# colmap/glomap

Measured on NVIDIA H100. Metric: observations/sec per BA LM-iteration, higher is better.
Workload: dtype f64

## Files before the change

### glomap_b200/csrc/ba_kernels.cuh

```cuda
#pragma once
#include "common.cuh"
#include "pcg.cuh"

namespace b200 {

constexpr int kCamRec = 8;
constexpr int kIntrRec = 8;
constexpr double kZEps = 1e-12;
constexpr int kSeg = 256;
constexpr int kIntrSmem = 16;
constexpr int kJpDoubles = 6;
constexpr int kSensorRec = 16;

struct BAView {
  int C, P, K;
  long long N;
  int n_tiles;
  int n_segs;
  int min_views;
  const int* obs_cam;
  const int* obs_pt;
  const double2* obs_xy;
  const unsigned* pt_begin;
  const int* tile_pt_begin;
// ... 22 lines not shown
  double* Dc;
};

__device__ __forceinline__ void huber(double s, double a, double& rho0, double& rho1) {
  const double b = a * a;
  if (s > b) {
    const double r = sqrt(s);
    rho0 = 2.0 * a * r - b;
    rho1 = fmax(2.2250738585072014e-308, a / r);
  } else {
    rho0 = s;
    rho1 = 1.0;
  }
}

__device__ __forceinline__ void project_jac(const double* __restrict__ ir, double x, double y, double z, double& px,
                                            double& py, double J[6]) {
  const double iz = 1.0 / z;
  const double u = x * iz, v = y * iz;
  const double fx = ir[0], fy = ir[1], cx = ir[2], cy = ir[3], k1 = ir[4], k2 = ir[5];
  const double r2 = u * u + v * v;
  const double d = 1.0 + r2 * (k1 + k2 * r2);
  const double dd = k1 + 2.0 * k2 * r2;
  px = fx * u * d + cx;
  py = fy * v * d + cy;
  const double a00 = d + 2.0 * u * u * dd, a01 = 2.0 * u * v * dd, a11 = d + 2.0 * v * v * dd;
  J[0] = fx * a00 * iz;
  J[1] = fx * a01 * iz;
  J[2] = -fx * iz * (a00 * u + a01 * v);
  J[3] = fy * a01 * iz;
  J[4] = fy * a11 * iz;
  J[5] = -fy * iz * (a01 * u + a11 * v);
}
__device__ __forceinline__ void project_only(const double* __restrict__ ir, double x, double y, double z, double& px,
                                             double& py) {
  const double iz = 1.0 / z;
  const double u = x * iz, v = y * iz;
  const double r2 = u * u + v * v;
  const double d = 1.0 + r2 * (ir[4] + ir[5] * r2);
  px = ir[0] * u * d + ir[2];
  py = ir[1] * v * d + ir[3];
}

struct ObsLin {
  double Jr[6], Jt[6], Jp[6], r[2], rho0;
  double u, v, w;
  bool valid;
};

__device__ __forceinline__ int cam_rec_intr(const double4& t4) { return (int)(__double_as_longlong(t4.w) >> 8); }

__device__ __forceinline__ void sensor_apply(const double* __restrict__ sr, double& x, double& y, double& z) {
  const double a = sr[0] * x + sr[1] * y + sr[2] * z + sr[9];
  const double b = sr[3] * x + sr[4] * y + sr[5] * z + sr[10];
  const double c = sr[6] * x + sr[7] * y + sr[8] * z + sr[11];
  x = a; y = b; z = c;
// ... 59 lines not shown
  for (int a = 0; a < 2; ++a) {
    const double j0 = J[3 * a], j1 = J[3 * a + 1], j2 = J[3 * a + 2];
    o.Jr[3 * a + 0] = rvar ? -2.0 * (j1 * rz - j2 * ry) : 0.0;
    o.Jr[3 * a + 1] = rvar ? -2.0 * (j2 * rx - j0 * rz) : 0.0;
    o.Jr[3 * a + 2] = rvar ? -2.0 * (j0 * ry - j1 * rx) : 0.0;
  }
#pragma unroll
  for (int a = 0; a < 2; ++a)
#pragma unroll
    for (int b = 0; b < 3; ++b) o.Jp[3 * a + b] = J[3 * a] * R[b] + J[3 * a + 1] * R[3 + b] + J[3 * a + 2] * R[6 + b];
}

struct ObsCore {
  double J[6], e[2], rho0, rho1, RX[3], R[9];
  double uv[2];
  bool valid;
};
__device__ __forceinline__ void obs_core(const double4& q4, const double4& t4, const double* __restrict__ ir,
                                         const double* __restrict__ sr, double X0, double X1, double X2, double2 xy,
                                         double huber_a, ObsCore& o) {
  const double q[4] = {q4.x, q4.y, q4.z, q4.w};
  quat_to_R(q, o.R);
  o.RX[0] = o.R[0] * X0 + o.R[1] * X1 + o.R[2] * X2;
  o.RX[1] = o.R[3] * X0 + o.R[4] * X1 + o.R[5] * X2;
  o.RX[2] = o.R[6] * X0 + o.R[7] * X1 + o.R[8] * X2;
  double xc = o.RX[0] + t4.x, yc = o.RX[1] + t4.y, zc = o.RX[2] + t4.z;
  if (sr) sensor_apply(sr, xc, yc, zc);
  o.valid = zc > kZEps;
  if (!o.valid) {
#pragma unroll
    for (int k = 0; k < 6; ++k) o.J[k] = 0.0;
    o.e[0] = o.e[1] = 0.0;
    o.rho0 = 0.0;
    o.rho1 = 0.0;
    o.uv[0] = o.uv[1] = 0.0;
    return;
  }
  double px, py;
  project_jac(ir, xc, yc, zc, px, py, o.J);
  o.uv[0] = xc / zc;
  o.uv[1] = yc / zc;
  if (sr) {
#pragma unroll
    for (int a = 0; a < 2; ++a) {
      const double j0 = o.J[3 * a], j1 = o.J[3 * a + 1], j2 = o.J[3 * a + 2];
      o.J[3 * a] = j0 * sr[0] + j1 * sr[3] + j2 * sr[6];
      o.J[3 * a + 1] = j0 * sr[1] + j1 * sr[4] + j2 * sr[7];
      o.J[3 * a + 2] = j0 * sr[2] + j1 * sr[5] + j2 * sr[8];
    }
  }
  o.e[0] = px - xy.x;
  o.e[1] = py - xy.y;
  const double s = o.e[0] * o.e[0] + o.e[1] * o.e[1];
  const double b = huber_a * huber_a;
  if (s > b) {
    const double t = rsqrt(s);
    o.rho1 = fmax(2.2250738585072014e-308, huber_a * t);
    o.rho0 = 2.0 * huber_a * (s * t) - b;
  } else {
    o.rho0 = s;
    o.rho1 = 1.0;
  }
}
__device__ __forceinline__ void obs_point_blocks(const ObsCore& o, double Jp[6], double A[6], double b[3]) {
#pragma unroll
  for (int a = 0; a < 2; ++a)
#pragma unroll
    for (int c = 0; c < 3; ++c) Jp[3 * a + c] = o.J[3 * a] * o.R[c] + o.J[3 * a + 1] * o.R[3 + c] + o.J[3 * a + 2] * o.R[6 + c];
  const double s0 = o.rho1 * Jp[0], s1 = o.rho1 * Jp[1], s2 = o.rho1 * Jp[2];
  const double s3 = o.rho1 * Jp[3], s4 = o.rho1 * Jp[4], s5 = o.rho1 * Jp[5];
  A[0] = s0 * Jp[0] + s3 * Jp[3];
  A[1] = s0 * Jp[1] + s3 * Jp[4];
  A[2] = s0 * Jp[2] + s3 * Jp[5];
  A[3] = s1 * Jp[1] + s4 * Jp[4];
  A[4] = s1 * Jp[2] + s4 * Jp[5];
  A[5] = s2 * Jp[2] + s5 * Jp[5];
  b[0] = s0 * o.e[0] + s3 * o.e[1];
// ... 672 lines not shown
    atomicAdd(&cscal[3], a3);
    atomicAdd(&cscal[4], a4);
  }
}


constexpr int kMaxBlockDof = 5;

struct IntrVarRec {
  int col0;
  int mb;
  int pidx[kMaxBlockDof];
  int pad;
};

__device__ __forceinline__ void intr_param_jac(const double* __restrict__ ir, int pidx, double u, double v, double w,
                                               double& jx, double& jy) {
  const int model = (int)ir[6];
  const double r2 = u * u + v * v;
  const double d = 1.0 + r2 * (ir[4] + ir[5] * r2);
  jx = 0.0;
  jy = 0.0;
  if (model == 1) {
    if (pidx == 0) jx = u;
    else if (pidx == 1) jy = v;
    else if (pidx == 2) jx = 1.0;
    else jy = 1.0;
  } else {
    if (pidx == 0) { jx = u * d; jy = v * d; }
    else if (pidx == 1) jx = 1.0;
    else if (pidx == 2) jy = 1.0;
    else if (pidx == 3) { jx = ir[0] * u * r2; jy = ir[1] * v * r2; }
    else { jx = ir[0] * u * r2 * r2; jy = ir[1] * v * r2 * r2; }
  }
  jx *= w;
  jy *= w;
}

__global__ void __launch_bounds__(256) ba_colsum(int rows, int ncol, const double* __restrict__ part,
                                                 double* __restrict__ out) {
  __shared__ double scratch[32];
  const int c = blockIdx.x;
  double a = 0.0;
  for (int r = threadIdx.x; r < rows; r += blockDim.x) a += part[(size_t)r * ncol + c];
  a = block_sum(a, scratch);
  if (threadIdx.x == 0) out[c] = a;
}

// ... 2 lines not shown
```

### glomap_b200/csrc/ba_kernels_ext.cuh

```cuda
#pragma once
#include "ba_kernels_v3.cuh"

namespace b200 {

struct ExtView {
  int C, K, S;
  const IntrVarRec* ivar;
  const unsigned char* sensor_var;
};

template <bool WK, bool WS>
struct ObsFull {
  double Jr[6], Jt[6], Jp[6], r[2], rho0;
  double Jk[WK ? 2 : 1][kMaxBlockDof];
  double Jsr[WS ? 6 : 1], Jst[WS ? 6 : 1];
  bool valid;
};

template <bool WK, bool WS>
__device__ __forceinline__ void obs_full(const double4& q4, const double4& t4, const double* __restrict__ ir,
                                         const IntrVarRec& iv, const double* __restrict__ sr, bool svar, double X0,
                                         double X1, double X2, double2 xy, double huber_a, ObsFull<WK, WS>& o) {
  const int mask = (int)(__double_as_longlong(t4.w) & 0xff);
  const double q[4] = {q4.x, q4.y, q4.z, q4.w};
// ... 35 lines not shown
#pragma unroll
      for (int a = 0; a < 2; ++a) {
        const double j0 = J[3 * a], j1 = J[3 * a + 1], j2 = J[3 * a + 2];
        o.Jsr[WS ? 3 * a + 0 : 0] = -2.0 * (j1 * a2 - j2 * a1);
        o.Jsr[WS ? 3 * a + 1 : 0] = -2.0 * (j2 * a0 - j0 * a2);
        o.Jsr[WS ? 3 * a + 2 : 0] = -2.0 * (j0 * a1 - j1 * a0);
        o.Jst[WS ? 3 * a + 0 : 0] = j0;
        o.Jst[WS ? 3 * a + 1 : 0] = j1;
        o.Jst[WS ? 3 * a + 2 : 0] = j2;
      }
    }
  }
  if (WK) {
#pragma unroll
    for (int j = 0; j < kMaxBlockDof; ++j)
      if (j < iv.mb) intr_param_jac(ir, iv.pidx[j], u, v, w, o.Jk[0][j], o.Jk[WK ? 1 : 0][j]);
  }
  if (sr) {
#pragma unroll
    for (int a = 0; a < 2; ++a) {
      const double j0 = J[3 * a], j1 = J[3 * a + 1], j2 = J[3 * a + 2];
      J[3 * a] = j0 * sr[0] + j1 * sr[3] + j2 * sr[6];
      J[3 * a + 1] = j0 * sr[1] + j1 * sr[4] + j2 * sr[7];
      J[3 * a + 2] = j0 * sr[2] + j1 * sr[5] + j2 * sr[8];
    }
  }
  const bool tvar = !(mask & 2), rvar = !(mask & 1);
#pragma unroll
  for (int a = 0; a < 2; ++a) {
    const double j0 = J[3 * a], j1 = J[3 * a + 1], j2 = J[3 * a + 2];
    if (tvar) { o.Jt[3 * a] = j0; o.Jt[3 * a + 1] = j1; o.Jt[3 * a + 2] = j2; }
// ... 391 lines not shown
```

### glomap_b200/csrc/ba_kernels_v2.cuh

```cuda
#pragma once
#include "ba_kernels.cuh"
#include "pcg.cuh"

namespace b200 {

struct BAViewV2 {
  const double* Ap;
  double* z4;
  const double* pts4;
  double* Ufk = nullptr;
  const IntrVarRec* ivar = nullptr;
  int C = 0;
};

template <int NK>
__device__ __forceinline__ void obs_intr_rows(const ObsCore& o, const double* __restrict__ ir, const IntrVarRec& iv,
                                              const double Jp[6], double Jk[2][NK > 0 ? NK : 1],
                                              double B[NK > 0 ? 3 * NK : 1]) {
#pragma unroll
  for (int j = 0; j < NK; ++j) {
    double jx = 0.0, jy = 0.0;
    if (j < iv.mb) intr_param_jac(ir, iv.pidx[j], o.uv[0], o.uv[1], 1.0, jx, jy);
    if (!o.valid) jx = jy = 0.0;
    Jk[0][j] = jx;
    Jk[1][j] = jy;
#pragma unroll
    for (int c = 0; c < 3; ++c) B[3 * j + c] = o.rho1 * (Jp[c] * jx + Jp[3 + c] * jy);
  }
}

constexpr int kXqStride = 8;
__global__ void ba2_pack_x(int C, const double* __restrict__ x, const double* __restrict__ cam_rec,
                           double* __restrict__ xp) {
  const int c = blockIdx.x * blockDim.x + threadIdx.x;
  if (c >= C) return;
  const double* r = cam_rec + (size_t)c * kCamRec;
  const double q[4] = {r[0], r[1], r[2], r[3]};
  double R[9];
  quat_to_R(q, R);
  const double* xc = x + (size_t)c * 6;
  double* o = xp + (size_t)c * kXqStride;
#pragma unroll
  for (int k = 0; k < 3; ++k) {
// ... 40 lines not shown
__global__ void ba2_pad_points(int P, const double* __restrict__ points, double* __restrict__ pts4) {
  const int p = blockIdx.x * blockDim.x + threadIdx.x;
  if (p >= P) return;
  const double x = points[3 * (size_t)p], y = points[3 * (size_t)p + 1], z = points[3 * (size_t)p + 2];
  st_rec32(pts4 + 4 * (size_t)p, x, y, z, 0.0);
}

template <int NK>
__global__ void __launch_bounds__(128, NK > 0 ? 3 : B200_LC_MIN_CTAS) ba2_linearize_cams(BAView v, BAViewV2 v2, const double* __restrict__ cam_rec,
                                                         const double* __restrict__ intr_rec, double huber_a) {
  const int warp = (blockIdx.x * blockDim.x + threadIdx.x) >> 5;
  const int lane = threadIdx.x & 31;
  if (warp >= v.n_segs) return;
  const int cam = v.seg_cam[warp];
  const int b = v.seg_begin[warp], e = v.seg_end[warp];
  const double4 q4c = ld_rec32(cam_rec + (size_t)cam * kCamRec);
  const double4 t4c = ld_rec32(cam_rec + (size_t)cam * kCamRec + 4);
  const double* irc = intr_rec + (size_t)v.seg_intr[warp] * kIntrRec;
  const double* src = sensor_of_seg(v, warp);
  double U[21], g[6];
#pragma unroll
  for (int k = 0; k < 21; ++k) U[k] = 0.0;
#pragma unroll
  for (int k = 0; k < 6; ++k) g[k] = 0.0;
  const int cmask = (int)(__double_as_longlong(t4c.w) & 0xff);
  const bool tvar = !(cmask & 2), rvar = !(cmask & 1);
  constexpr int NKK = NK > 0 ? NK : 1;
  const int blk = v.seg_intr[warp];
  IntrVarRec iv{};
  if (NK > 0) iv = v2.ivar[blk];
  double Ukk[NKK * (NKK + 1) / 2], gk[NKK], Ufk[6][NKK];
#pragma unroll
  for (int k = 0; k < NKK * (NKK + 1) / 2; ++k) Ukk[k] = 0.0;
#pragma unroll
  for (int k = 0; k < NKK; ++k) {
    gk[k] = 0.0;
#pragma unroll
    for (int i2 = 0; i2 < 6; ++i2) Ufk[i2][k] = 0.0;
  }
  const double* __restrict__ pts4 = v2.pts4;
// ... 6 lines not shown
    if (i + 32 < e) pt_nxt = ld_stream(v.pt_c + i + 32);
    xy = ld_stream(v.xy_c + i);
    Xc = ld_rec32(pts4 + 4 * (size_t)pt0);
  }
  for (; i < e; i += 32) {
    double4 Xn = Xc;
    double2 xyn = xy;
    int pt_nn = 0;
    if (i + 32 < e) {
      Xn = ld_rec32(pts4 + 4 * (size_t)pt_nxt);
      xyn = ld_stream(v.xy_c + i + 32);
    }
    if (i + 64 < e) pt_nn = ld_stream(v.pt_c + i + 64);
    const double X0 = Xc.x, X1 = Xc.y, X2 = Xc.z;
    ObsCore o;
    obs_core(q4c, t4c, irc, src, X0, X1, X2, xy, huber_a, o);
    double Jp[6], A[6], bo[3];
    obs_point_blocks(o, Jp, A, bo);
    double Jc[2][6];
#pragma unroll
    for (int a = 0; a < 2; ++a) {
      const double j0 = o.J[3 * a], j1 = o.J[3 * a + 1], j2 = o.J[3 * a + 2];
      Jc[a][0] = rvar ? -2.0 * (j1 * o.RX[2] - j2 * o.RX[1]) : 0.0;
      Jc[a][1] = rvar ? -2.0 * (j2 * o.RX[0] - j0 * o.RX[2]) : 0.0;
      Jc[a][2] = rvar ? -2.0 * (j0 * o.RX[1] - j1 * o.RX[0]) : 0.0;
      Jc[a][3] = tvar ? j0 : 0.0;
      Jc[a][4] = tvar ? j1 : 0.0;
      Jc[a][5] = tvar ? j2 : 0.0;
    }
    const double e0 = o.rho1 * o.e[0], e1 = o.rho1 * o.e[1];
    int idx = 0;
#pragma unroll
    for (int i2 = 0; i2 < 6; ++i2) {
      const double s0 = o.rho1 * Jc[0][i2], s1 = o.rho1 * Jc[1][i2];
#pragma unroll
      for (int j = i2; j < 6; ++j) U[idx++] += s0 * Jc[0][j] + s1 * Jc[1][j];
      g[i2] += Jc[0][i2] * e0 + Jc[1][i2] * e1;
    }
    if (NK > 0) {
      double Jk[2][NKK], Bo[3 * NKK];
      obs_intr_rows<NK>(o, irc, iv, Jp, Jk, Bo);
      int ik = 0;
#pragma unroll
      for (int a = 0; a < NK; ++a) {
        const double s0 = o.rho1 * Jk[0][a], s1 = o.rho1 * Jk[1][a];
#pragma unroll
        for (int c = a; c < NK; ++c) Ukk[ik++] += s0 * Jk[0][c] + s1 * Jk[1][c];
        gk[a] += Jk[0][a] * e0 + Jk[1][a] * e1;
#pragma unroll
        for (int i2 = 0; i2 < 6; ++i2) Ufk[i2][a] += Jc[0][i2] * s0 + Jc[1][i2] * s1;
      }
    }
    Xc = Xn; xy = xyn; pt_nxt = pt_nn;
  }
  if (NK > 0) {
    const size_t kb = (size_t)(v2.C + blk);
// ... 14 lines not shown
      }
    }
  }
#pragma unroll
  for (int k = 0; k < 21; ++k) {
    const double s = warp_sum(U[k]);
    if (lane == k && s != 0.0) atomicAdd(&v.U[(size_t)cam * 21 + k], s);
  }
#pragma unroll
  for (int k = 0; k < 6; ++k) {
    const double s = warp_sum(g[k]);
    if (lane == 21 + k && s != 0.0) atomicAdd(&v.gc[(size_t)cam * 6 + k], s);
  }
}

__global__ void __launch_bounds__(128) ba2_schur_diag(BAView v, BAViewV2 v2, const double* __restrict__ cam_rec,
                                                      const double* __restrict__ intr_rec, double huber_a) {
  const int warp = (blockIdx.x * blockDim.x + threadIdx.x) >> 5;
  const int lane = threadIdx.x & 31;
  if (warp >= v.n_segs) return;
  const int cam = v.seg_cam[warp];
  const int b = v.seg_begin[warp], e = v.seg_end[warp];
  const double4 q4c = ld_rec32(cam_rec + (size_t)cam * kCamRec);
  const double4 t4c = ld_rec32(cam_rec + (size_t)cam * kCamRec + 4);
  const double* irc = intr_rec + (size_t)v.seg_intr[warp] * kIntrRec;
  const double* src = sensor_of_seg(v, warp);
  double RR[6] = {0, 0, 0, 0, 0, 0}, RT[9] = {0, 0, 0, 0, 0, 0, 0, 0, 0}, TT[6] = {0, 0, 0, 0, 0, 0};
  int i = b + lane;
  int pt_nxt = 0;
  double2 xy = make_double2(0, 0), va = xy, vb = xy, vc = xy;
  double4 Xc = make_double4(0, 0, 0, 0);
  if (i < e) {
    const int pt0 = ld_stream(v.pt_c + i);
    if (i + 32 < e) pt_nxt = ld_stream(v.pt_c + i + 32);
    xy = ld_stream(v.xy_c + i);
    Xc = ld_rec32(v2.pts4 + 4 * (size_t)pt0);
    const double2* vp = reinterpret_cast<const double2*>(v.Vinv + (size_t)pt0 * 6);
    va = vp[0]; vb = vp[1]; vc = vp[2];
  }
  for (; i < e; i += 32) {
    double4 Xn = Xc;
    double2 xyn = xy, van = va, vbn = vb, vcn = vc;
    int pt_nn = 0;
    if (i + 32 < e) {
      Xn = ld_rec32(v2.pts4 + 4 * (size_t)pt_nxt);
      xyn = ld_stream(v.xy_c + i + 32);
      const double2* vp = reinterpret_cast<const double2*>(v.Vinv + (size_t)pt_nxt * 6);
      van = vp[0]; vbn = vp[1]; vcn = vp[2];
    }
    if (i + 64 < e) pt_nn = ld_stream(v.pt_c + i + 64);
    const double X[3] = {Xc.x, Xc.y, Xc.z};
    ObsCore o;
    obs_core(q4c, t4c, irc, src, X[0], X[1], X[2], xy, huber_a, o);
    double Jp[6], A[6], bo[3];
    obs_point_blocks(o, Jp, A, bo);
    const double vi[6] = {va.x, va.y, vb.x, vb.y, vc.x, vc.y};
    const double Ac0[3] = {A[0], A[1], A[2]}, Ac1[3] = {A[1], A[3], A[4]}, Ac2[3] = {A[2], A[4], A[5]};
    double T0[3], T1[3], T2[3];
    sym3_mul(vi, Ac0, T0);
    sym3_mul(vi, Ac1, T1);
    sym3_mul(vi, Ac2, T2);
    double N[3][3];
    {
      double c0[3], c1[3], c2[3];
      sym3_mul(A, T0, c0);
      sym3_mul(A, T1, c1);
      sym3_mul(A, T2, c2);
#pragma unroll
      for (int r = 0; r < 3; ++r) { N[r][0] = c0[r]; N[r][1] = c1[r]; N[r][2] = c2[r]; }
    }
    double P[3][3];
#pragma unroll
    for (int c = 0; c < 3; ++c) {
      const double n0 = N[0][c], n1 = N[1][c], n2 = N[2][c];
      P[0][c] = 2.0 * (X[1] * n2 - X[2] * n1);
      P[1][c] = 2.0 * (X[2] * n0 - X[0] * n2);
      P[2][c] = 2.0 * (X[0] * n1 - X[1] * n0);
    }
    double PK[3][3];
#pragma unroll
    for (int r = 0; r < 3; ++r) {
      PK[r][0] = P[r][1] * X[2] - P[r][2] * X[1];
      PK[r][1] = -P[r][0] * X[2] + P[r][2] * X[0];
      PK[r][2] = P[r][0] * X[1] - P[r][1] * X[0];
    }
// ... 1 lines not shown
    RR[3] += -2.0 * PK[1][1]; RR[4] += -2.0 * PK[1][2]; RR[5] += -2.0 * PK[2][2];
#pragma unroll
    for (int r = 0; r < 3; ++r)
#pragma unroll
      for (int c = 0; c < 3; ++c) RT[3 * r + c] += P[r][c];
    TT[0] += N[0][0]; TT[1] += N[0][1]; TT[2] += N[0][2]; TT[3] += N[1][1]; TT[4] += N[1][2]; TT[5] += N[2][2];
    Xc = Xn; xy = xyn; va = van; vb = vbn; vc = vcn; pt_nxt = pt_nn;
  }
#pragma unroll
  for (int k = 0; k < 6; ++k) RR[k] = warp_sum(RR[k]);
#pragma unroll
  for (int k = 0; k < 9; ++k) RT[k] = warp_sum(RT[k]);
#pragma unroll
  for (int k = 0; k < 6; ++k) TT[k] = warp_sum(TT[k]);
  if (lane == 0) {
    const int mask = (int)(__double_as_longlong(t4c.w) & 0xff);
    const double q[4] = {q4c.x, q4c.y, q4c.z, q4c.w};
    double R[9];
    quat_to_R(q, R);
    double M[6][6];
    const double rr[3][3] = {{RR[0], RR[1], RR[2]}, {RR[1], RR[3], RR[4]}, {RR[2], RR[4], RR[5]}};
    const double tt[3][3] = {{TT[0], TT[1], TT[2]}, {TT[1], TT[3], TT[4]}, {TT[2], TT[4], TT[5]}};
    for (int r = 0; r < 3; ++r)
      for (int c = 0; c < 3; ++c) {
        M[r][c] = rr[r][c];
        M[3 + r][3 + c] = tt[r][c];
        M[r][3 + c] = RT[3 * r + c];
        M[3 + c][r] = RT[3 * r + c];
      }
    double T[6][6];
    for (int blk = 0; blk < 2; ++blk)
      for (int r = 0; r < 3; ++r)
        for (int c = 0; c < 6; ++c)
          T[3 * blk + r][c] = R[3 * r] * M[3 * blk][c] + R[3 * r + 1] * M[3 * blk + 1][c] + R[3 * r + 2] * M[3 * blk + 2][c];
// ... 194 lines not shown
  const bool pvalid = (int)(v.pt_begin[p + 1] - v.pt_begin[p]) >= v.min_views;
  *reinterpret_cast<double4*>(v2.z4 + 4 * (size_t)p) = pvalid ? make_double4(z[0], z[1], z[2], 0.0) : make_double4(0, 0, 0, 0);
}

template <int NK>
__global__ void __launch_bounds__(128, B200_PB_MIN_CTAS) ba2_pass_b(BAView v, BAViewV2 v2, const double* __restrict__ cam_rec,
                                                 const double* __restrict__ intr_rec, double huber_a,
                                                 double* __restrict__ y, const PcgCtl* __restrict__ ctl, int seg_lo,
                                                 int seg_hi) {
  if (ctl && ctl->done) return;
  const int warp = seg_lo + ((blockIdx.x * blockDim.x + threadIdx.x) >> 5);
  const int lane = threadIdx.x & 31;
  if (warp >= seg_hi) return;
  const int cam = v.seg_cam[warp];
  const int b = v.seg_begin[warp], e = v.seg_end[warp];
  const double4 q4c = ld_rec32(cam_rec + (size_t)cam * kCamRec);
  const double4 t4c = ld_rec32(cam_rec + (size_t)cam * kCamRec + 4);
  const int blk = v.seg_intr[warp];
  const double* irc = intr_rec + (size_t)blk * kIntrRec;
  const double* src = sensor_of_seg(v, warp);
  constexpr int NKK = NK > 0 ? NK : 1;
  IntrVarRec iv{};
  if (NK > 0) iv = v2.ivar[blk];
  double acc[6] = {0, 0, 0, 0, 0, 0};
  double accK[NKK];
#pragma unroll
  for (int k = 0; k < NKK; ++k) accK[k] = 0.0;
  const uint64_t keep = l2_policy_evict_last();
  int i = b + lane;
  int pt_nxt = 0;
  double4 X = make_double4(0, 0, 0, 0), z = X;
  double2 xy = make_double2(0, 0);
  if (i < e) {
    const int pt0 = ld_stream(v.pt_c + i);
    if (i + 32 < e) pt_nxt = ld_stream(v.pt_c + i + 32);
    X = ld_rec32(v2.pts4 + 4 * (size_t)pt0);
    z = ld_keep4(v2.z4 + 4 * (size_t)pt0, keep);
    xy = ld_stream(v.xy_c + i);
  }
  for (; i < e; i += 32) {
    double4 Xn = X, zn = z;
    double2 xyn = xy;
    int pt_nn = 0;
    if (i + 32 < e) {
      Xn = ld_rec32(v2.pts4 + 4 * (size_t)pt_nxt);
      zn = ld_keep4(v2.z4 + 4 * (size_t)pt_nxt, keep);
      xyn = ld_stream(v.xy_c + i + 32);
    }
    if (i + 64 < e) pt_nn = ld_stream(v.pt_c + i + 64);
    ObsCore o;
    obs_core(q4c, t4c, irc, src, X.x, X.y, X.z, xy, huber_a, o);
    double Jp[6], a[6], bo[3];
    obs_point_blocks(o, Jp, a, bo);
    const double w0 = a[0] * z.x + a[1] * z.y + a[2] * z.z;
    const double w1 = a[1] * z.x + a[3] * z.y + a[4] * z.z;
    const double w2 = a[2] * z.x + a[4] * z.y + a[5] * z.z;
    acc[0] += 2.0 * (X.y * w2 - X.z * w1);
    acc[1] += 2.0 * (X.z * w0 - X.x * w2);
    acc[2] += 2.0 * (X.x * w1 - X.y * w0);
    acc[3] += w0;
    acc[4] += w1;
    acc[5] += w2;
    if (NK > 0) {
      double Jk[2][NKK], Bo[3 * NKK];
      obs_intr_rows<NK>(o, irc, iv, Jp, Jk, Bo);
#pragma unroll
      for (int k = 0; k < NK; ++k) accK[k] += Bo[3 * k] * z.x + Bo[3 * k + 1] * z.y + Bo[3 * k + 2] * z.z;
    }
    X = Xn; z = zn; xy = xyn; pt_nxt = pt_nn;
  }
#pragma unroll
  for (int k = 0; k < 6; ++k) acc[k] = warp_sum(acc[k]);
  if (lane < 6) {
    const int mask = (int)(__double_as_longlong(t4c.w) & 0xff);
    const double q[4] = {q4c.x, q4c.y, q4c.z, q4c.w};
    double R[9];
    quat_to_R(q, R);
    const int bl = lane / 3, r = lane % 3;
    const bool fixed = bl == 0 ? (mask & 1) : (mask & 2);
    const double s = R[3 * r] * acc[3 * bl] + R[3 * r + 1] * acc[3 * bl + 1] + R[3 * r + 2] * acc[3 * bl + 2];
    if (!fixed && s != 0.0) atomicAdd(&y[(size_t)cam * 6 + lane], -s);
  }
  if (NK > 0) {
    const size_t kb = (size_t)(v2.C + blk);
#pragma unroll
    for (int k = 0; k < NK; ++k) {
      const double sk = warp_sum(accK[k]);
      if (lane == 0 && sk != 0.0) atomicAdd(&y[kb * 6 + k], -sk);
    }
  }
}

__global__ void ba2k_pack_xk(int C, const double* __restrict__ cam_rec, const double* __restrict__ x, double* __restrict__ xp,
                             const PcgCtl* __restrict__ ctl) {
  if (ctl && ctl->done) return;
  const int c = blockIdx.x * blockDim.x + threadIdx.x;
// ... 57 lines not shown
```

### glomap_b200/csrc/ba_kernels_v3.cuh

```cuda
#pragma once
#include "ba_kernels_v2.cuh"

namespace b200 {

constexpr int kEllWindow = 1024;
constexpr int kEllThreads = 128;

struct EllView {
  int n_groups;
  const int* row0;
  const int* pt;
  const int* len;
  const int* cam;
  const double2* xy;
  const unsigned short* sensor;
  double* A;
  double* B = nullptr;
};

template <class Sort>
__global__ void __launch_bounds__(kEllWindow) ell_sort_window(int P, int min_views, const unsigned* __restrict__ pt_begin,
                                                              int* __restrict__ ell_pt, int* __restrict__ ell_len,
                                                              int* __restrict__ ell_slot, int* __restrict__ group_rows) {
  __shared__ typename Sort::TempStorage tmp;
// ... 115 lines not shown
      obs_core(qA, tA, ir, sr, X0, X1, X2, xyA, huber_a, o);
      cost += 0.5 * o.rho0;
      if (points_var) {
        double Jp[6], A[6], b[3];
        obs_point_blocks(o, Jp, A, b);
        double* row = ell.A + ((size_t)r0 + j) * (6 * 32) + lane;
#pragma unroll
        for (int k = 0; k < 6; ++k) {
          st_stream(row + 32 * k, A[k]);
          V[k] += A[k];
        }
        gp[0] += b[0]; gp[1] += b[1]; gp[2] += b[2];
        if (NK > 0) {
          constexpr int NKK = NK > 0 ? NK : 1;
          double Jk[2][NKK], Bo[3 * NKK];
          obs_intr_rows<NK>(o, ir, ivar[blk], Jp, Jk, Bo);
          double* rowB = ell.B + ((size_t)r0 + j) * (3 * NK * 32) + lane;
#pragma unroll
          for (int k = 0; k < 3 * NK; ++k) st_stream(rowB + 32 * k, Bo[k]);
        }
      }
#if B200_E1_PIPE >= 2
      qA = qB; tA = tB; qB2 = qC; tB2 = tC; xyA = xyB; xyB = xyC; camC2 = camD;
#else
      qA = qB; tA = tB; xyA = xyB; xyB = xyC; camB = camC;
#endif
    }
#else
#pragma unroll 2
    for (int j = 0; j < nrow; ++j) {
      if (j >= mylen) continue;
// ... 9 lines not shown
      obs_core(q4, t4, ir, sr, X0, X1, X2, xy, huber_a, o);
      cost += 0.5 * o.rho0;
      if (points_var) {
        double Jp[6], A[6], b[3];
        obs_point_blocks(o, Jp, A, b);
        double* row = ell.A + ((size_t)r0 + j) * (6 * 32) + lane;
#pragma unroll
        for (int k = 0; k < 6; ++k) {
          st_stream(row + 32 * k, A[k]);
          V[k] += A[k];
        }
        gp[0] += b[0]; gp[1] += b[1]; gp[2] += b[2];
        if (NK > 0) {
          constexpr int NKK = NK > 0 ? NK : 1;
          double Jk[2][NKK], Bo[3 * NKK];
          obs_intr_rows<NK>(o, ir, ivar[blk], Jp, Jk, Bo);
          double* rowB = ell.B + ((size_t)r0 + j) * (3 * NK * 32) + lane;
#pragma unroll
          for (int k = 0; k < 3 * NK; ++k) st_stream(rowB + 32 * k, Bo[k]);
        }
      }
    }
#endif
    if (points_var && pt >= 0) {
#pragma unroll
      for (int k = 0; k < 6; ++k) v.V[6 * (size_t)pt + k] = V[k];
#pragma unroll
      for (int k = 0; k < 3; ++k) {
        v.gp[3 * (size_t)pt + k] = gp[k];
        gmax = fmax(gmax, fabs(gp[k]));
      }
// ... 180 lines not shown
```

### glomap_b200/csrc/common.cuh

```cuda
#pragma once
#include <cuda_runtime.h>
#include <stdint.h>
#include <stdio.h>

#include <string>

namespace b200 {

#ifndef B200_TILE
#define B200_TILE 128
#endif
#ifndef B200_K1_MIN_CTAS
#define B200_K1_MIN_CTAS 5
#endif
#ifndef B200_K3_MIN_CTAS
#define B200_K3_MIN_CTAS 8
#endif
#ifndef B200_PA_MIN_CTAS
#define B200_PA_MIN_CTAS 12
#endif
#ifndef B200_LC_MIN_CTAS
#define B200_LC_MIN_CTAS 3
#endif
#ifndef B200_PB_MIN_CTAS
#define B200_PB_MIN_CTAS 4
#endif
#ifndef B200_E1_MIN_CTAS
#define B200_E1_MIN_CTAS 4
#endif
#ifndef B200_E1_PIPE
#define B200_E1_PIPE 1
#endif
#ifndef B200_EA_MIN_CTAS
#define B200_EA_MIN_CTAS 8
#endif
#ifndef B200_EA2_MIN_CTAS
#define B200_EA2_MIN_CTAS 6
#endif
#ifndef B200_STREAM_HINTS
#define B200_STREAM_HINTS 1
// ... 283 lines not shown
```

### profiles/sass_excerpt.py

```python
#!/usr/bin/env python
import collections
import os
import re
import subprocess

ROOT = os.path.dirname(os.path.dirname(os.path.abspath(__file__)))
KERNELS = ["ba3_linearize_points", "ba2_linearize_cams", "ba3_pass_a", "ba2_pass_b", "ba2_schur_diag", "ba3_cost",
           "ba2_pcg_direction_pack", "pcg_update", "pcg_apply_diag", "bax_pass_b", "ba2k_cross", "gp_schur_pass", "ra_laplacian_csr",
           "ra2_laplacian_dot", "ra2_coarse", "p2p_allreduce_sum", "proc_undistort", "trk_hook"]
KEEP = re.compile(r"^(LDG|STG|LDS|STS|RED|ATOM|BAR|SHFL|DFMA|DMUL|DADD|MUFU|CCTL|UBLKCP|SYNCS|MEMBAR|ERRBAR|LDGSTS)")


def main():
    lib = os.path.join(ROOT, "glomap_b200", "libb200sfm.so")
    txt = subprocess.run(["cuobjdump", "-sass", lib], capture_output=True, text=True).stdout
    names = subprocess.run(["cu++filt"], input="\n".join(re.findall(r"Function : (\S+)", txt)), capture_output=True, text=True).stdout.split("\n")
    mangled = re.findall(r"Function : (\S+)", txt)
    demangle = dict(zip(mangled, names))
    cur, counts, totals = None, collections.defaultdict(collections.Counter), collections.Counter()
    for line in txt.splitlines():
        m = re.search(r"Function : (\S+)", line)
        if m:
            cur = demangle.get(m.group(1), m.group(1))
            continue
        m = re.search(r"/\*[0-9a-f]{4}\*/\s+(?:@!?U?P\d+\s+)?([A-Z0-9_.]+)", line)
        if m and cur:
            totals[cur] += 1
            op = m.group(1)
            if KEEP.match(op):
                counts[cur][op] += 1
    print("# SASS mnemonics of the hot kernels (cuobjdump -sass glomap_b200/libb200sfm.so, sm_90a)")
    print("# per kernel: total instructions, then the memory / synchronisation / FP64 mnemonics with their static counts")
    print("# (profiles/sass_excerpt.py regenerates this file; no tensor-core or TMA mnemonics are expected: FP64 streaming kernels)\n")
    for k in sorted(counts):
        if not any(re.search(r"\b" + re.escape(n) + r"\b", k) for n in KERNELS):
            continue
        ops = ", ".join(f"{o} x{c}" for o, c in counts[k].most_common(14))
        print(k[:200])
        print(f"    total {totals[k]} instructions: {ops}")


if __name__ == "__main__":
    main()
```

Baseline: 1.405 billion.

## Hoist per-segment rotation and factor projection Jacobian to cut FP64 work in BA kernels

```diff
diff --git a/glomap_b200/csrc/ba_kernels.cuh b/glomap_b200/csrc/ba_kernels.cuh
--- a/glomap_b200/csrc/ba_kernels.cuh
+++ b/glomap_b200/csrc/ba_kernels.cuh
@@ -60,32 +60,69 @@
   }
 }
 
+struct Intr {
+  double fx, fy, cx, cy, k1, k2;
+  int model;
+};
+__device__ __forceinline__ Intr ld_intr(const double* __restrict__ ir) {
+  return Intr{ir[0], ir[1], ir[2], ir[3], ir[4], ir[5], (int)ir[6]};
+}
+
+struct ProjJac {
+  double iz, u, v, m00, m01, m10, m11;
+};
+
+__device__ __forceinline__ void project_jac(const Intr& in, double x, double y, double z, double& px, double& py,
+                                            ProjJac& pj) {
+  const double iz = 1.0 / z;
+  const double u = x * iz, v = y * iz;
+  pj.iz = iz;
+  pj.u = u;
+  pj.v = v;
+  if (in.k1 == 0.0 && in.k2 == 0.0) {
+    px = in.fx * u + in.cx;
+    py = in.fy * v + in.cy;
+    pj.m00 = in.fx; pj.m01 = 0.0; pj.m10 = 0.0; pj.m11 = in.fy;
+  } else {
+    const double r2 = u * u + v * v;
+    const double d = 1.0 + r2 * (in.k1 + in.k2 * r2);
+    const double dd = in.k1 + 2.0 * in.k2 * r2;
+    px = in.fx * u * d + in.cx;
+    py = in.fy * v * d + in.cy;
+    const double a00 = d + 2.0 * u * u * dd, a01 = 2.0 * u * v * dd, a11 = d + 2.0 * v * v * dd;
+    pj.m00 = in.fx * a00; pj.m01 = in.fx * a01; pj.m10 = in.fy * a01; pj.m11 = in.fy * a11;
+  }
+}
+__device__ __forceinline__ void project_only(const Intr& in, double x, double y, double z, double& px, double& py) {
+  const double iz = 1.0 / z;
+  const double u = x * iz, v = y * iz;
+  if (in.k1 == 0.0 && in.k2 == 0.0) {
+    px = in.fx * u + in.cx;
+    py = in.fy * v + in.cy;
+  } else {
+    const double r2 = u * u + v * v;
+    const double d = 1.0 + r2 * (in.k1 + in.k2 * r2);
+    px = in.fx * u * d + in.cx;
+    py = in.fy * v * d + in.cy;
+  }
+}
+__device__ __forceinline__ void proj_jac_rows(const ProjJac& pj, double J[6]) {
+  J[0] = pj.m00 * pj.iz;
+  J[1] = pj.m01 * pj.iz;
+  J[2] = -(J[0] * pj.u + J[1] * pj.v);
+  J[3] = pj.m10 * pj.iz;
+  J[4] = pj.m11 * pj.iz;
+  J[5] = -(J[3] * pj.u + J[4] * pj.v);
+}
 __device__ __forceinline__ void project_jac(const double* __restrict__ ir, double x, double y, double z, double& px,
                                             double& py, double J[6]) {
-  const double iz = 1.0 / z;
-  const double u = x * iz, v = y * iz;
-  const double fx = ir[0], fy = ir[1], cx = ir[2], cy = ir[3], k1 = ir[4], k2 = ir[5];
-  const double r2 = u * u + v * v;
-  const double d = 1.0 + r2 * (k1 + k2 * r2);
-  const double dd = k1 + 2.0 * k2 * r2;
-  px = fx * u * d + cx;
-  py = fy * v * d + cy;
-  const double a00 = d + 2.0 * u * u * dd, a01 = 2.0 * u * v * dd, a11 = d + 2.0 * v * v * dd;
-  J[0] = fx * a00 * iz;
-  J[1] = fx * a01 * iz;
-  J[2] = -fx * iz * (a00 * u + a01 * v);
-  J[3] = fy * a01 * iz;
-  J[4] = fy * a11 * iz;
-  J[5] = -fy * iz * (a01 * u + a11 * v);
+  ProjJac pj;
+  project_jac(ld_intr(ir), x, y, z, px, py, pj);
+  proj_jac_rows(pj, J);
 }
 __device__ __forceinline__ void project_only(const double* __restrict__ ir, double x, double y, double z, double& px,
                                              double& py) {
-  const double iz = 1.0 / z;
-  const double u = x * iz, v = y * iz;
-  const double r2 = u * u + v * v;
-  const double d = 1.0 + r2 * (ir[4] + ir[5] * r2);
-  px = ir[0] * u * d + ir[2];
-  py = ir[1] * v * d + ir[3];
+  project_only(ld_intr(ir), x, y, z, px, py);
 }
 
 struct ObsLin {
@@ -175,13 +212,14 @@
 struct ObsCore {
   double J[6], e[2], rho0, rho1, RX[3], R[9];
   double uv[2];
+  ProjJac pj;
   bool valid;
 };
-__device__ __forceinline__ void obs_core(const double4& q4, const double4& t4, const double* __restrict__ ir,
-                                         const double* __restrict__ sr, double X0, double X1, double X2, double2 xy,
-                                         double huber_a, ObsCore& o) {
-  const double q[4] = {q4.x, q4.y, q4.z, q4.w};
-  quat_to_R(q, o.R);
+__device__ __forceinline__ void obs_core_R(const double R[9], const double4& t4, const Intr& in,
+                                           const double* __restrict__ sr, double X0, double X1, double X2, double2 xy,
+                                           double huber_a, ObsCore& o) {
+#pragma unroll
+  for (int k = 0; k < 9; ++k) o.R[k] = R[k];
   o.RX[0] = o.R[0] * X0 + o.R[1] * X1 + o.R[2] * X2;
   o.RX[1] = o.R[3] * X0 + o.R[4] * X1 + o.R[5] * X2;
   o.RX[2] = o.R[6] * X0 + o.R[7] * X1 + o.R[8] * X2;
@@ -195,10 +233,12 @@
     o.rho0 = 0.0;
     o.rho1 = 0.0;
     o.uv[0] = o.uv[1] = 0.0;
+    o.pj = ProjJac{0.0, 0.0, 0.0, 0.0, 0.0, 0.0, 0.0};
     return;
   }
   double px, py;
-  project_jac(ir, xc, yc, zc, px, py, o.J);
+  project_jac(in, xc, yc, zc, px, py, o.pj);
+  proj_jac_rows(o.pj, o.J);
   o.uv[0] = xc / zc;
   o.uv[1] = yc / zc;
   if (sr) {
@@ -222,6 +262,14 @@
     o.rho0 = s;
     o.rho1 = 1.0;
   }
+}
+__device__ __forceinline__ void obs_core(const double4& q4, const double4& t4, const double* __restrict__ ir,
+                                         const double* __restrict__ sr, double X0, double X1, double X2, double2 xy,
+                                         double huber_a, ObsCore& o) {
+  const double q[4] = {q4.x, q4.y, q4.z, q4.w};
+  double R[9];
+  quat_to_R(q, R);
+  obs_core_R(R, t4, ld_intr(ir), sr, X0, X1, X2, xy, huber_a, o);
 }
 __device__ __forceinline__ void obs_point_blocks(const ObsCore& o, double Jp[6], double A[6], double b[3]) {
 #pragma unroll
@@ -924,14 +972,13 @@
   int pad;
 };
 
-__device__ __forceinline__ void intr_param_jac(const double* __restrict__ ir, int pidx, double u, double v, double w,
+__device__ __forceinline__ void intr_param_jac(const Intr& in, int pidx, double u, double v, double w,
                                                double& jx, double& jy) {
-  const int model = (int)ir[6];
   const double r2 = u * u + v * v;
-  const double d = 1.0 + r2 * (ir[4] + ir[5] * r2);
+  const double d = 1.0 + r2 * (in.k1 + in.k2 * r2);
   jx = 0.0;
   jy = 0.0;
-  if (model == 1) {
+  if (in.model == 1) {
     if (pidx == 0) jx = u;
     else if (pidx == 1) jy = v;
     else if (pidx == 2) jx = 1.0;
@@ -940,8 +987,8 @@
     if (pidx == 0) { jx = u * d; jy = v * d; }
     else if (pidx == 1) jx = 1.0;
     else if (pidx == 2) jy = 1.0;
-    else if (pidx == 3) { jx = ir[0] * u * r2; jy = ir[1] * v * r2; }
-    else { jx = ir[0] * u * r2 * r2; jy = ir[1] * v * r2 * r2; }
+    else if (pidx == 3) { jx = in.fx * u * r2; jy = in.fy * v * r2; }
+    else { jx = in.fx * u * r2 * r2; jy = in.fy * v * r2 * r2; }
   }
   jx *= w;
   jy *= w;
diff --git a/glomap_b200/csrc/ba_kernels_ext.cuh b/glomap_b200/csrc/ba_kernels_ext.cuh
--- a/glomap_b200/csrc/ba_kernels_ext.cuh
+++ b/glomap_b200/csrc/ba_kernels_ext.cuh
@@ -73,7 +73,7 @@
   if (WK) {
 #pragma unroll
     for (int j = 0; j < kMaxBlockDof; ++j)
-      if (j < iv.mb) intr_param_jac(ir, iv.pidx[j], u, v, w, o.Jk[0][j], o.Jk[WK ? 1 : 0][j]);
+      if (j < iv.mb) intr_param_jac(ld_intr(ir), iv.pidx[j], u, v, w, o.Jk[0][j], o.Jk[WK ? 1 : 0][j]);
   }
   if (sr) {
 #pragma unroll
diff --git a/glomap_b200/csrc/ba_kernels_v2.cuh b/glomap_b200/csrc/ba_kernels_v2.cuh
--- a/glomap_b200/csrc/ba_kernels_v2.cuh
+++ b/glomap_b200/csrc/ba_kernels_v2.cuh
@@ -14,19 +14,64 @@
 };
 
 template <int NK>
-__device__ __forceinline__ void obs_intr_rows(const ObsCore& o, const double* __restrict__ ir, const IntrVarRec& iv,
-                                              const double Jp[6], double Jk[2][NK > 0 ? NK : 1],
-                                              double B[NK > 0 ? 3 * NK : 1]) {
+__device__ __forceinline__ void obs_intr_jac(const ObsCore& o, const Intr& in, const IntrVarRec& iv,
+                                             double Jk[2][NK > 0 ? NK : 1]) {
 #pragma unroll
   for (int j = 0; j < NK; ++j) {
     double jx = 0.0, jy = 0.0;
-    if (j < iv.mb) intr_param_jac(ir, iv.pidx[j], o.uv[0], o.uv[1], 1.0, jx, jy);
+    if (j < iv.mb) intr_param_jac(in, iv.pidx[j], o.uv[0], o.uv[1], 1.0, jx, jy);
     if (!o.valid) jx = jy = 0.0;
     Jk[0][j] = jx;
     Jk[1][j] = jy;
-#pragma unroll
-    for (int c = 0; c < 3; ++c) B[3 * j + c] = o.rho1 * (Jp[c] * jx + Jp[3 + c] * jy);
-  }
+  }
+}
+template <int NK>
+__device__ __forceinline__ void obs_intr_rows(const ObsCore& o, const Intr& in, const IntrVarRec& iv,
+                                              const double Jp[6], double Jk[2][NK > 0 ? NK : 1],
+                                              double B[NK > 0 ? 3 * NK : 1]) {
+  obs_intr_jac<NK>(o, in, iv, Jk);
+#pragma unroll
+  for (int j = 0; j < NK; ++j)
+#pragma unroll
+    for (int c = 0; c < 3; ++c) B[3 * j + c] = o.rho1 * (Jp[c] * Jk[0][j] + Jp[3 + c] * Jk[1][j]);
+}
+
+struct SegRec {
+  double R[9];
+  double4 t4;
+  Intr in;
+  const double* sr;
+};
+__device__ __forceinline__ void seg_records(const BAView& v, int seg, int cam, const double* __restrict__ cam_rec,
+                                            const double* __restrict__ intr_rec, SegRec& s) {
+  const double4 q4 = ld_rec32(cam_rec + (size_t)cam * kCamRec);
+  s.t4 = ld_rec32(cam_rec + (size_t)cam * kCamRec + 4);
+  s.in = ld_intr(intr_rec + (size_t)v.seg_intr[seg] * kIntrRec);
+  s.sr = sensor_of_seg(v, seg);
+  const double q[4] = {q4.x, q4.y, q4.z, q4.w};
+  quat_to_R(q, s.R);
+}
+__device__ __forceinline__ void to_sensor(const double* __restrict__ sr, double x[3]) {
+  if (!sr) return;
+  const double x0 = x[0], x1 = x[1], x2 = x[2];
+#pragma unroll
+  for (int k = 0; k < 3; ++k) x[k] = sr[3 * k] * x0 + sr[3 * k + 1] * x1 + sr[3 * k + 2] * x2;
+}
+__device__ __forceinline__ void cam_frame_jac(const ObsCore& o, const double r[3], double a[2], double w[3]) {
+  const ProjJac& p = o.pj;
+  const double t0 = r[0] - p.u * r[2], t1 = r[1] - p.v * r[2];
+  const double c = o.rho1 * p.iz;
+  a[0] = c * (p.m00 * t0 + p.m01 * t1);
+  a[1] = c * (p.m10 * t0 + p.m11 * t1);
+  const double s0 = p.iz * (p.m00 * a[0] + p.m10 * a[1]), s1 = p.iz * (p.m01 * a[0] + p.m11 * a[1]);
+  w[0] = s0;
+  w[1] = s1;
+  w[2] = -(p.u * s0 + p.v * s1);
+}
+__device__ __forceinline__ void rig_to_frame(const double* __restrict__ sr, double x[3]) {
+  const double x0 = x[0], x1 = x[1], x2 = x[2];
+#pragma unroll
+  for (int k = 0; k < 3; ++k) x[k] = sr[k] * x0 + sr[3 + k] * x1 + sr[6 + k] * x2;
 }
 
 constexpr int kXqStride = 8;
@@ -97,16 +142,14 @@
   if (warp >= v.n_segs) return;
   const int cam = v.seg_cam[warp];
   const int b = v.seg_begin[warp], e = v.seg_end[warp];
-  const double4 q4c = ld_rec32(cam_rec + (size_t)cam * kCamRec);
-  const double4 t4c = ld_rec32(cam_rec + (size_t)cam * kCamRec + 4);
-  const double* irc = intr_rec + (size_t)v.seg_intr[warp] * kIntrRec;
-  const double* src = sensor_of_seg(v, warp);
+  SegRec sg;
+  seg_records(v, warp, cam, cam_rec, intr_rec, sg);
   double U[21], g[6];
 #pragma unroll
   for (int k = 0; k < 21; ++k) U[k] = 0.0;
 #pragma unroll
   for (int k = 0; k < 6; ++k) g[k] = 0.0;
-  const int cmask = (int)(__double_as_longlong(t4c.w) & 0xff);
+  const int cmask = (int)(__double_as_longlong(sg.t4.w) & 0xff);
   const bool tvar = !(cmask & 2), rvar = !(cmask & 1);
   constexpr int NKK = NK > 0 ? NK : 1;
   const int blk = v.seg_intr[warp];
@@ -143,9 +186,7 @@
     if (i + 64 < e) pt_nn = ld_stream(v.pt_c + i + 64);
     const double X0 = Xc.x, X1 = Xc.y, X2 = Xc.z;
     ObsCore o;
-    obs_core(q4c, t4c, irc, src, X0, X1, X2, xy, huber_a, o);
-    double Jp[6], A[6], bo[3];
-    obs_point_blocks(o, Jp, A, bo);
+    obs_core_R(sg.R, sg.t4, sg.in, sg.sr, X0, X1, X2, xy, huber_a, o);
     double Jc[2][6];
 #pragma unroll
     for (int a = 0; a < 2; ++a) {
@@ -167,8 +208,8 @@
       g[i2] += Jc[0][i2] * e0 + Jc[1][i2] * e1;
     }
     if (NK > 0) {
-      double Jk[2][NKK], Bo[3 * NKK];
-      obs_intr_rows<NK>(o, irc, iv, Jp, Jk, Bo);
+      double Jk[2][NKK];
+      obs_intr_jac<NK>(o, sg.in, iv, Jk);
       int ik = 0;
 #pragma unroll
       for (int a = 0; a < NK; ++a) {
@@ -213,17 +254,15 @@
   }
 }
 
-__global__ void __launch_bounds__(128) ba2_schur_diag(BAView v, BAViewV2 v2, const double* __restrict__ cam_rec,
-                                                      const double* __restrict__ intr_rec, double huber_a) {
+__global__ void __launch_bounds__(128, B200_SD_MIN_CTAS) ba2_schur_diag(BAView v, BAViewV2 v2, const double* __restrict__ cam_rec,
+                                                                        const double* __restrict__ intr_rec, double huber_a) {
   const int warp = (blockIdx.x * blockDim.x + threadIdx.x) >> 5;
   const int lane = threadIdx.x & 31;
   if (warp >= v.n_segs) return;
   const int cam = v.seg_cam[warp];
   const int b = v.seg_begin[warp], e = v.seg_end[warp];
-  const double4 q4c = ld_rec32(cam_rec + (size_t)cam * kCamRec);
-  const double4 t4c = ld_rec32(cam_rec + (size_t)cam * kCamRec + 4);
-  const double* irc = intr_rec + (size_t)v.seg_intr[warp] * kIntrRec;
-  const double* src = sensor_of_seg(v, warp);
+  SegRec sg;
+  seg_records(v, warp, cam, cam_rec, intr_rec, sg);
   double RR[6] = {0, 0, 0, 0, 0, 0}, RT[9] = {0, 0, 0, 0, 0, 0, 0, 0, 0}, TT[6] = {0, 0, 0, 0, 0, 0};
   int i = b + lane;
   int pt_nxt = 0;
@@ -248,26 +287,42 @@
       van = vp[0]; vbn = vp[1]; vcn = vp[2];
     }
     if (i + 64 < e) pt_nn = ld_stream(v.pt_c + i + 64);
-    const double X[3] = {Xc.x, Xc.y, Xc.z};
     ObsCore o;
-    obs_core(q4c, t4c, irc, src, X[0], X[1], X[2], xy, huber_a, o);
-    double Jp[6], A[6], bo[3];
-    obs_point_blocks(o, Jp, A, bo);
+    obs_core_R(sg.R, sg.t4, sg.in, sg.sr, Xc.x, Xc.y, Xc.z, xy, huber_a, o);
+    double X[3] = {o.RX[0], o.RX[1], o.RX[2]};
+    to_sensor(sg.sr, X);
+    const ProjJac& pj = o.pj;
     const double vi[6] = {va.x, va.y, vb.x, vb.y, vc.x, vc.y};
-    const double Ac0[3] = {A[0], A[1], A[2]}, Ac1[3] = {A[1], A[3], A[4]}, Ac2[3] = {A[2], A[4], A[5]};
-    double T0[3], T1[3], T2[3];
-    sym3_mul(vi, Ac0, T0);
-    sym3_mul(vi, Ac1, T1);
-    sym3_mul(vi, Ac2, T2);
+    double e0[3] = {1.0, 0.0, -pj.u}, e1[3] = {0.0, 1.0, -pj.v};
+    if (sg.sr) {
+#pragma unroll
+      for (int c = 0; c < 3; ++c) {
+        e0[c] = sg.sr[c] - pj.u * sg.sr[6 + c];
+        e1[c] = sg.sr[3 + c] - pj.v * sg.sr[6 + c];
+      }
+    }
+    double l0[3], l1[3], t0[3], t1[3];
+#pragma unroll
+    for (int c = 0; c < 3; ++c) {
+      l0[c] = e0[0] * sg.R[c] + e0[1] * sg.R[3 + c] + e0[2] * sg.R[6 + c];
+      l1[c] = e1[0] * sg.R[c] + e1[1] * sg.R[3 + c] + e1[2] * sg.R[6 + c];
+    }
+    sym3_mul(vi, l0, t0);
+    sym3_mul(vi, l1, t1);
+    const double q00 = l0[0] * t0[0] + l0[1] * t0[1] + l0[2] * t0[2];
+    const double q01 = l0[0] * t1[0] + l0[1] * t1[1] + l0[2] * t1[2];
+    const double q11 = l1[0] * t1[0] + l1[1] * t1[1] + l1[2] * t1[2];
+    const double k00 = pj.m00 * pj.m00 + pj.m10 * pj.m10, k01 = pj.m00 * pj.m01 + pj.m10 * pj.m11,
+                 k11 = pj.m01 * pj.m01 + pj.m11 * pj.m11;
+    const double a00 = k00 * q00 + k01 * q01, a01 = k00 * q01 + k01 * q11;
+    const double a10 = k01 * q00 + k11 * q01, a11 = k01 * q01 + k11 * q11;
+    const double sc = o.rho1 * pj.iz * pj.iz, c2 = sc * sc;
+    const double h00 = c2 * (a00 * k00 + a01 * k01), h01 = c2 * (a00 * k01 + a01 * k11), h11 = c2 * (a10 * k01 + a11 * k11);
     double N[3][3];
-    {
-      double c0[3], c1[3], c2[3];
-      sym3_mul(A, T0, c0);
-      sym3_mul(A, T1, c1);
-      sym3_mul(A, T2, c2);
-#pragma unroll
-      for (int r = 0; r < 3; ++r) { N[r][0] = c0[r]; N[r][1] = c1[r]; N[r][2] = c2[r]; }
-    }
+    N[0][0] = h00; N[0][1] = N[1][0] = h01; N[1][1] = h11;
+    N[0][2] = N[2][0] = -(h00 * pj.u + h01 * pj.v);
+    N[1][2] = N[2][1] = -(h01 * pj.u + h11 * pj.v);
+    N[2][2] = -(N[0][2] * pj.u + N[1][2] * pj.v);
     double P[3][3];
 #pragma unroll
     for (int c = 0; c < 3; ++c) {
@@ -299,10 +354,12 @@
 #pragma unroll
   for (int k = 0; k < 6; ++k) TT[k] = warp_sum(TT[k]);
   if (lane == 0) {
-    const int mask = (int)(__double_as_longlong(t4c.w) & 0xff);
-    const double q[4] = {q4c.x, q4c.y, q4c.z, q4c.w};
-    double R[9];
-    quat_to_R(q, R);
+    const int mask = (int)(__double_as_longlong(sg.t4.w) & 0xff);
+    double R[9] = {1, 0, 0, 0, 1, 0, 0, 0, 1};
+    if (sg.sr) {
+      for (int r = 0; r < 3; ++r)
+        for (int c = 0; c < 3; ++c) R[3 * r + c] = sg.sr[3 * c + r];
+    }
     double M[6][6];
     const double rr[3][3] = {{RR[0], RR[1], RR[2]}, {RR[1], RR[3], RR[4]}, {RR[2], RR[4], RR[5]}};
     const double tt[3][3] = {{TT[0], TT[1], TT[2]}, {TT[1], TT[3], TT[4]}, {TT[2], TT[4], TT[5]}};
@@ -527,11 +584,9 @@
   if (warp >= seg_hi) return;
   const int cam = v.seg_cam[warp];
   const int b = v.seg_begin[warp], e = v.seg_end[warp];
-  const double4 q4c = ld_rec32(cam_rec + (size_t)cam * kCamRec);
-  const double4 t4c = ld_rec32(cam_rec + (size_t)cam * kCamRec + 4);
   const int blk = v.seg_intr[warp];
-  const double* irc = intr_rec + (size_t)blk * kIntrRec;
-  const double* src = sensor_of_seg(v, warp);
+  SegRec sg;
+  seg_records(v, warp, cam, cam_rec, intr_rec, sg);
   constexpr int NKK = NK > 0 ? NK : 1;
   IntrVarRec iv{};
   if (NK > 0) iv = v2.ivar[blk];
@@ -562,37 +617,41 @@
     }
     if (i + 64 < e) pt_nn = ld_stream(v.pt_c + i + 64);
     ObsCore o;
-    obs_core(q4c, t4c, irc, src, X.x, X.y, X.z, xy, huber_a, o);
-    double Jp[6], a[6], bo[3];
-    obs_point_blocks(o, Jp, a, bo);
-    const double w0 = a[0] * z.x + a[1] * z.y + a[2] * z.z;
-    const double w1 = a[1] * z.x + a[3] * z.y + a[4] * z.z;
-    const double w2 = a[2] * z.x + a[4] * z.y + a[5] * z.z;
-    acc[0] += 2.0 * (X.y * w2 - X.z * w1);
-    acc[1] += 2.0 * (X.z * w0 - X.x * w2);
-    acc[2] += 2.0 * (X.x * w1 - X.y * w0);
-    acc[3] += w0;
-    acc[4] += w1;
-    acc[5] += w2;
+    obs_core_R(sg.R, sg.t4, sg.in, sg.sr, X.x, X.y, X.z, xy, huber_a, o);
+    double P[3] = {o.RX[0], o.RX[1], o.RX[2]};
+    to_sensor(sg.sr, P);
+    double r[3] = {sg.R[0] * z.x + sg.R[1] * z.y + sg.R[2] * z.z,
+                   sg.R[3] * z.x + sg.R[4] * z.y + sg.R[5] * z.z,
+                   sg.R[6] * z.x + sg.R[7] * z.y + sg.R[8] * z.z};
+    to_sensor(sg.sr, r);
+    double a[2], w[3];
+    cam_frame_jac(o, r, a, w);
+    acc[0] += P[1] * w[2] - P[2] * w[1];
+    acc[1] += P[2] * w[0] - P[0] * w[2];
+    acc[2] += P[0] * w[1] - P[1] * w[0];
+    acc[3] += w[0];
+    acc[4] += w[1];
+    acc[5] += w[2];
     if (NK > 0) {
-      double Jk[2][NKK], Bo[3 * NKK];
-      obs_intr_rows<NK>(o, irc, iv, Jp, Jk, Bo);
-#pragma unroll
-      for (int k = 0; k < NK; ++k) accK[k] += Bo[3 * k] * z.x + Bo[3 * k + 1] * z.y + Bo[3 * k + 2] * z.z;
+      double Jk[2][NKK];
+      obs_intr_jac<NK>(o, sg.in, iv, Jk);
+#pragma unroll
+      for (int k = 0; k < NK; ++k) accK[k] += Jk[0][k] * a[0] + Jk[1][k] * a[1];
     }
     X = Xn; z = zn; xy = xyn; pt_nxt = pt_nn;
   }
 #pragma unroll
   for (int k = 0; k < 6; ++k) acc[k] = warp_sum(acc[k]);
-  if (lane < 6) {
-    const int mask = (int)(__double_as_longlong(t4c.w) & 0xff);
-    const double q[4] = {q4c.x, q4c.y, q4c.z, q4c.w};
-    double R[9];
-    quat_to_R(q, R);
-    const int bl = lane / 3, r = lane % 3;
-    const bool fixed = bl == 0 ? (mask & 1) : (mask & 2);
-    const double s = R[3 * r] * acc[3 * bl] + R[3 * r + 1] * acc[3 * bl + 1] + R[3 * r + 2] * acc[3 * bl + 2];
-    if (!fixed && s != 0.0) atomicAdd(&y[(size_t)cam * 6 + lane], -s);
+  if (sg.sr) {
+    rig_to_frame(sg.sr, acc);
+    rig_to_frame(sg.sr, acc + 3);
+  }
+  const int mask = (int)(__double_as_longlong(sg.t4.w) & 0xff);
+#pragma unroll
+  for (int k = 0; k < 6; ++k) {
+    const double s = k < 3 ? 2.0 * acc[k] : acc[k];
+    const bool fixed = k < 3 ? (mask & 1) : (mask & 2);
+    if (lane == k && !fixed && s != 0.0) atomicAdd(&y[(size_t)cam * 6 + k], -s);
   }
   if (NK > 0) {
     const size_t kb = (size_t)(v2.C + blk);
diff --git a/glomap_b200/csrc/ba_kernels_v3.cuh b/glomap_b200/csrc/ba_kernels_v3.cuh
--- a/glomap_b200/csrc/ba_kernels_v3.cuh
+++ b/glomap_b200/csrc/ba_kernels_v3.cuh
@@ -153,7 +153,7 @@
         if (NK > 0) {
           constexpr int NKK = NK > 0 ? NK : 1;
           double Jk[2][NKK], Bo[3 * NKK];
-          obs_intr_rows<NK>(o, ir, ivar[blk], Jp, Jk, Bo);
+          obs_intr_rows<NK>(o, ld_intr(ir), ivar[blk], Jp, Jk, Bo);
           double* rowB = ell.B + ((size_t)r0 + j) * (3 * NK * 32) + lane;
 #pragma unroll
           for (int k = 0; k < 3 * NK; ++k) st_stream(rowB + 32 * k, Bo[k]);
@@ -193,7 +193,7 @@
         if (NK > 0) {
           constexpr int NKK = NK > 0 ? NK : 1;
           double Jk[2][NKK], Bo[3 * NKK];
-          obs_intr_rows<NK>(o, ir, ivar[blk], Jp, Jk, Bo);
+          obs_intr_rows<NK>(o, ld_intr(ir), ivar[blk], Jp, Jk, Bo);
           double* rowB = ell.B + ((size_t)r0 + j) * (3 * NK * 32) + lane;
 #pragma unroll
           for (int k = 0; k < 3 * NK; ++k) st_stream(rowB + 32 * k, Bo[k]);
diff --git a/glomap_b200/csrc/common.cuh b/glomap_b200/csrc/common.cuh
--- a/glomap_b200/csrc/common.cuh
+++ b/glomap_b200/csrc/common.cuh
@@ -24,6 +24,9 @@
 #endif
 #ifndef B200_PB_MIN_CTAS
 #define B200_PB_MIN_CTAS 4
+#endif
+#ifndef B200_SD_MIN_CTAS
+#define B200_SD_MIN_CTAS 3
 #endif
 #ifndef B200_E1_MIN_CTAS
 #define B200_E1_MIN_CTAS 4
diff --git a/profiles/sass_excerpt.py b/profiles/sass_excerpt.py
--- a/profiles/sass_excerpt.py
+++ b/profiles/sass_excerpt.py
@@ -9,6 +9,24 @@
            "ba2_pcg_direction_pack", "pcg_update", "pcg_apply_diag", "bax_pass_b", "ba2k_cross", "gp_schur_pass", "ra_laplacian_csr",
            "ra2_laplacian_dot", "ra2_coarse", "p2p_allreduce_sum", "proc_undistort", "trk_hook"]
 KEEP = re.compile(r"^(LDG|STG|LDS|STS|RED|ATOM|BAR|SHFL|DFMA|DMUL|DADD|MUFU|CCTL|UBLKCP|SYNCS|MEMBAR|ERRBAR|LDGSTS)")
+LOOP_KERNELS = ["ba2_pass_b", "ba2_schur_diag", "ba2_linearize_cams", "ba3_pass_a"]
+FP64 = re.compile(r"^(DFMA|DMUL|DADD|DSETP|DMNMX|MUFU)")
+LOADS = re.compile(r"^(LDG|LD|LDS|LDL|LDC)\b")
+INSN = re.compile(r"/\*([0-9a-f]{4,})\*/\s+(?:@!?U?P\w+\s+)?([A-Z0-9_.]+)([^;]*);")
+
+
+def inner_loop(insns):
+    best = None
+    for addr, op, args in insns:
+        m = re.search(r"0x([0-9a-f]+)\s*$", args.strip())
+        if op.startswith("BRA") and m and int(m.group(1), 16) < addr:
+            body = [(a, o) for a, o, _ in insns if int(m.group(1), 16) <= a <= addr]
+            if best is None or len(body) > len(best):
+                best = body
+    if not best:
+        return None
+    ops = [o for _, o in best]
+    return len(ops), sum(bool(FP64.match(o)) for o in ops), sum(bool(LOADS.match(o)) for o in ops)
 
 
 def main():
@@ -18,15 +36,17 @@
     mangled = re.findall(r"Function : (\S+)", txt)
     demangle = dict(zip(mangled, names))
     cur, counts, totals = None, collections.defaultdict(collections.Counter), collections.Counter()
+    insns = collections.defaultdict(list)
     for line in txt.splitlines():
         m = re.search(r"Function : (\S+)", line)
         if m:
             cur = demangle.get(m.group(1), m.group(1))
             continue
-        m = re.search(r"/\*[0-9a-f]{4}\*/\s+(?:@!?U?P\d+\s+)?([A-Z0-9_.]+)", line)
+        m = INSN.search(line)
         if m and cur:
             totals[cur] += 1
-            op = m.group(1)
+            op = m.group(2)
+            insns[cur].append((int(m.group(1), 16), op, m.group(3)))
             if KEEP.match(op):
                 counts[cur][op] += 1
     print("# SASS mnemonics of the hot kernels (cuobjdump -sass glomap_b200/libb200sfm.so, sm_90a)")
@@ -38,6 +58,10 @@
         ops = ", ".join(f"{o} x{c}" for o, c in counts[k].most_common(14))
         print(k[:200])
         print(f"    total {totals[k]} instructions: {ops}")
+        if any(re.search(r"\b" + n + r"\b", k) for n in LOOP_KERNELS):
+            loop = inner_loop(insns[k])
+            if loop:
+                print(f"    inner loop: {loop[0]} instructions, {loop[1]} FP64 + MUFU, {loop[2]} loads")
 
 
 if __name__ == "__main__":
```

New measurement: 1.504 billion, median of 6. 7.1% higher.
